# wenyuqing/panacea

Hardware: NVIDIA H100
Metric: UNet denoise-steps/s (6-view x 8-frame latent, CFG-doubled eps-eval + guidance + Euler update) (higher is better)
Workload: dtype bf16

## Files before the change

panacea_b200/csrc/attn_fa.cu:

```cuda
#include "common.cuh"
#include "ptx.cuh"
#include "operand.cuh"
#include "../../include/panacea_b200.h"

namespace pn {

constexpr int FA_THREADS = 288;
constexpr int FA_TILE_BYTES = 128 * 128;
constexpr int FA_XTILE_BYTES = 128 * 32;
constexpr int FA_MAX_KEYS = 128;

template <int D>
struct FaL {
  static constexpr int STAGES = 3;
  static constexpr int XB = D == 64 ? 0 : FA_XTILE_BYTES;
  static constexpr int Q = 0;
  static constexpr int QX = FA_TILE_BYTES;
  static constexpr int KV = FA_TILE_BYTES + XB;
  static constexpr int STAGE_BYTES = 2 * FA_TILE_BYTES + 2 * XB;
  static constexpr int BAR = KV + STAGES * STAGE_BYTES;
  static constexpr int TOTAL = BAR + 128 + 1024;
};

struct FaParams {
  CUtensorMap mapQ;
  CUtensorMap mapK;
  CUtensorMap mapV;
  CUtensorMap mapQx, mapKx, mapVx;
  int heads;
  int F, H, V, W;
  int qw, qh, tiles_x, tiles_y;
  int tiles_per_group;
  int kw, kh, kv_rows, kv_yblocks;
  int kv_views[8][2];
  int kv_view_count[8];
  int kv_frame_div;
  float scale_log2;
  __nv_bfloat16* out;
  long long out_ld;
};

template <int D>
__global__ void __launch_bounds__(FA_THREADS, 1) attn_fa_kernel(const __grid_constant__ FaParams p) {
  using L = FaL<D>;
  constexpr int STAGES = L::STAGES;
  extern __shared__ uint8_t smem_raw[];
  uint8_t* smem = smem_align1024(smem_raw);
  uint64_t* bars = reinterpret_cast<uint64_t*>(smem + L::BAR);
  uint64_t* q_full = bars;
  uint64_t* kv_full = bars + 1;
  uint64_t* kv_empty = bars + 1 + STAGES;

  const int warp = threadIdx.x >> 5;
  const int lane = threadIdx.x & 31;

  {
    uint4* z = reinterpret_cast<uint4*>(smem);
    for (int i = threadIdx.x; i < L::BAR / 16; i += FA_THREADS) z[i] = make_uint4(0, 0, 0, 0);
    fence_proxy_async_smem();
  }
  if (threadIdx.x == 0) {
    mbar_init(q_full, 1);
    for (int i = 0; i < STAGES; ++i) { mbar_init(&kv_full[i], 1); mbar_init(&kv_empty[i], 2); }
    fence_barrier_init();
  }
  __syncthreads();

  int item = blockIdx.x;
  const int ti = item % p.tiles_per_group; item /= p.tiles_per_group;
  const int head = item % p.heads; item /= p.heads;
  const int view = item % p.V;
  const int frame = item / p.V;
  const int nblk = p.kv_view_count[view] * p.kv_yblocks;

  if (warp == 8) {
    const uint32_t q_bytes = (uint32_t)(p.qw * p.qh) * (D == 80 ? 160u : 128u);
    const uint32_t kv_bytes = (uint32_t)p.kv_rows * (D == 80 ? 160u : 128u);
    if (elect_one()) {
      tma_prefetch_desc(&p.mapQ);
      tma_prefetch_desc(&p.mapK);
      tma_prefetch_desc(&p.mapV);
      mbar_arrive_expect_tx(q_full, q_bytes);
      const int x0 = (ti % p.tiles_x) * p.qw, y0 = (ti / p.tiles_x) * p.qh;
      tma_load_5d(smem + L::Q, &p.mapQ, q_full, head * D, x0, view, y0, frame);
      if (D == 80) tma_load_5d(smem + L::QX, &p.mapQx, q_full, head * D + 64, x0, view, y0, frame);
    }
    const int kv_frame = frame / p.kv_frame_div;
    int vi = 0, yb = 0;
    for (int j = 0; j < nblk; ++j) {
      const int st = j % STAGES;
      const int kvv = p.kv_views[view][vi];
      mbar_wait(&kv_empty[st], (uint32_t)(((j / STAGES) & 1) ^ 1));
      if (elect_one()) {
        uint8_t* sK = smem + L::KV + st * L::STAGE_BYTES;
        mbar_arrive_expect_tx(&kv_full[st], 2 * kv_bytes);
        tma_load_5d(sK, &p.mapK, &kv_full[st], head * D, 0, kvv, yb * p.kh, kv_frame);
        tma_load_5d(sK + FA_TILE_BYTES, &p.mapV, &kv_full[st], head * D, 0, kvv, yb * p.kh, kv_frame);
        if (D == 80) {
          tma_load_5d(sK + 2 * FA_TILE_BYTES, &p.mapKx, &kv_full[st], head * D + 64, 0, kvv, yb * p.kh, kv_frame);
          tma_load_5d(sK + 2 * FA_TILE_BYTES + L::XB, &p.mapVx, &kv_full[st], head * D + 64, 0, kvv, yb * p.kh, kv_frame);
        }
      }
      if (++yb == p.kv_yblocks) { yb = 0; ++vi; }
    }
    return;
  }

  const int wg = warp >> 2;
  const int quad = lane & 3;
  const uint32_t base = smem_u32(smem);
  const uint64_t dQ = wgmma_desc(base + L::Q + wg * 64 * 128, 16, 1024, kSw128);
  const uint64_t dQx = wgmma_desc(base + L::QX + wg * 64 * 32, 16, 256, kSw32);
  const uint64_t dK0 = wgmma_desc(base + L::KV, 16, 1024, kSw128);
  const uint64_t dV0 = wgmma_desc(base + L::KV + FA_TILE_BYTES, 1024, 1024, kSw128);
  const uint64_t dKx0 = wgmma_desc(base + L::KV + 2 * FA_TILE_BYTES, 16, 256, kSw32);
  const uint64_t dVx0 = wgmma_desc(base + L::KV + 2 * FA_TILE_BYTES + L::XB, 256, 256, kSw32);
  constexpr uint64_t STAGE_STEP = L::STAGE_BYTES >> 4;
  const float c = p.scale_log2;
  const bool mask = p.kv_rows < FA_MAX_KEYS;

  float o[32], ox[8];
#pragma unroll
  for (int i = 0; i < 32; ++i) o[i] = 0.f;
#pragma unroll
  for (int i = 0; i < 8; ++i) ox[i] = 0.f;
  float m_run[2] = {-INFINITY, -INFINITY}, l_run[2] = {0.f, 0.f};

  mbar_wait(q_full, 0);
  for (int j = 0; j < nblk; ++j) {
    const int st = j % STAGES;
    mbar_wait(&kv_full[st], (uint32_t)((j / STAGES) & 1));
    float s[64];
    wgmma_fence();
#pragma unroll
    for (int k = 0; k < 4; ++k) wgmma_ss<128>(s, dQ + 2 * k, dK0 + STAGE_STEP * st + 2 * k, k > 0 ? 1u : 0u);
    if (D == 80) wgmma_ss<128>(s, dQx, dKx0 + STAGE_STEP * st, 1u);
    wgmma_commit();
    wgmma_wait<0>();
    wgmma_fence_regs(s);

    float mx[2] = {-INFINITY, -INFINITY};
#pragma unroll
    for (int jj = 0; jj < 16; ++jj) {
#pragma unroll
      for (int e = 0; e < 4; ++e) {
        float v = s[4 * jj + e] * c;
        if (mask && 8 * jj + 2 * quad + (e & 1) >= p.kv_rows) v = -INFINITY;
        s[4 * jj + e] = v;
        mx[e >> 1] = fmaxf(mx[e >> 1], v);
      }
    }
    float alpha[2];
#pragma unroll
    for (int h = 0; h < 2; ++h) {
      mx[h] = fmaxf(mx[h], __shfl_xor_sync(0xffffffffu, mx[h], 1));
      mx[h] = fmaxf(mx[h], __shfl_xor_sync(0xffffffffu, mx[h], 2));
      const float m_new = fmaxf(m_run[h], mx[h]);
      alpha[h] = ex2_approx(m_run[h] - m_new);
      m_run[h] = m_new;
    }
    float rs[2] = {0.f, 0.f};
    uint32_t pa[8][4];
#pragma unroll
    for (int jj = 0; jj < 16; ++jj) {
#pragma unroll
      for (int h = 0; h < 2; ++h) {
        const float e0 = ex2_approx(s[4 * jj + 2 * h] - m_run[h]);
        const float e1 = ex2_approx(s[4 * jj + 2 * h + 1] - m_run[h]);
        rs[h] += e0 + e1;
        pa[jj >> 1][(jj & 1) * 2 + h] = pack_bf16x2(e0, e1);
      }
    }
#pragma unroll
    for (int h = 0; h < 2; ++h) l_run[h] = l_run[h] * alpha[h] + rs[h];
#pragma unroll
    for (int jj = 0; jj < 8; ++jj) {
#pragma unroll
      for (int e = 0; e < 4; ++e) o[4 * jj + e] *= alpha[e >> 1];
    }
    if (D == 80) {
#pragma unroll
      for (int e = 0; e < 8; ++e) ox[e] *= alpha[(e >> 1) & 1];
    }

    wgmma_fence();
#pragma unroll
    for (int kk = 0; kk < 8; ++kk) {
      wgmma_rs_tb<64>(o, pa[kk], dV0 + STAGE_STEP * st + kk * (2048 >> 4), 1u);
      if (D == 80) wgmma_rs_tb<16>(ox, pa[kk], dVx0 + STAGE_STEP * st + kk * (512 >> 4), 1u);
    }
    wgmma_commit();
    wgmma_wait<0>();
    wgmma_fence_regs(o);
    if (D == 80) wgmma_fence_regs(ox);
    if ((threadIdx.x & 127) == 0) mbar_arrive(&kv_empty[st]);
  }

#pragma unroll
  for (int h = 0; h < 2; ++h) {
    float l = l_run[h];
    l += __shfl_xor_sync(0xffffffffu, l, 1);
    l += __shfl_xor_sync(0xffffffffu, l, 2);
    const float inv = 1.f / l;
    const int row = wg * 64 + (warp & 3) * 16 + (lane >> 2) + 8 * h;
    const int yy = row / p.qw, xx = row - yy * p.qw;
    const int x = (ti % p.tiles_x) * p.qw + xx, y = (ti / p.tiles_x) * p.qh + yy;
    if (row >= p.qw * p.qh || x >= p.W || y >= p.H) continue;
    const long long token = (((long long)frame * p.H + y) * p.V + view) * p.W + x;
    __nv_bfloat16* dst = p.out + token * p.out_ld + head * D + 2 * quad;
#pragma unroll
    for (int jj = 0; jj < 8; ++jj)
      *reinterpret_cast<uint32_t*>(dst + 8 * jj) = pack_bf16x2(o[4 * jj + 2 * h] * inv, o[4 * jj + 2 * h + 1] * inv);
    if (D == 80) {
#pragma unroll
      for (int jj = 0; jj < 2; ++jj)
        *reinterpret_cast<uint32_t*>(dst + 64 + 8 * jj) = pack_bf16x2(ox[4 * jj + 2 * h] * inv, ox[4 * jj + 2 * h + 1] * inv);
    }
  }
}

}

using namespace pn;

extern "C" int pn_attention(const pn_attn_args* a, int operand_mode, void* stream_v) {
  PN_OPERAND_MODES(Modes, operand_mode, "pn_attention", PN_OPERAND_BF16, PN_OPERAND_SPLIT3, PN_OPERAND_F32);
  if (operand_mode != PN_OPERAND_BF16) return attention_f32(a, operand_mode, stream_v);
  if (a == nullptr) return fail(PN_ERR_INVALID, "pn_attention: null args");
  PN_REQUIRE(a->q && a->k && a->v && a->out, "pn_attention: null tensor pointer");
  PN_REQUIRE(a->head_dim == 64 || a->head_dim == 80, "pn_attention: head_dim %d unsupported (64 or 80)", a->head_dim);
  const int FA_D = a->head_dim;
  PN_REQUIRE(a->heads > 0 && a->F > 0 && a->H > 0 && a->V > 0 && a->V <= 8 && a->W > 0, "pn_attention: bad query geometry");
  PN_REQUIRE(a->Hk > 0 && a->Vk > 0 && a->Vk <= 8 && a->Wk > 0 && a->kv_frame_div > 0, "pn_attention: bad key geometry");
  PN_REQUIRE(a->q_ld % 8 == 0 && a->kv_ld % 8 == 0 && a->out_ld % 8 == 0, "pn_attention: token strides must be multiples of 8");
  PN_REQUIRE(a->q_ld >= a->heads * FA_D && a->kv_ld >= a->heads * FA_D && a->out_ld >= a->heads * FA_D,
             "pn_attention: token stride smaller than heads*64");

  FaParams p;
  std::memset(&p, 0, sizeof(p));
  p.heads = a->heads;
  p.F = (int)a->F; p.H = (int)a->H; p.V = (int)a->V; p.W = (int)a->W;
  p.qw = (int)(a->W <= 128 ? a->W : 128);
  p.qh = 128 / p.qw;
  if (p.qh > a->H) p.qh = (int)a->H;
  if (p.qh < 1) p.qh = 1;
  p.tiles_x = (int)((a->W + p.qw - 1) / p.qw);
  p.tiles_y = (int)((a->H + p.qh - 1) / p.qh);
  PN_REQUIRE(a->Wk <= FA_MAX_KEYS, "pn_attention: key view width %lld > %d unsupported", (long long)a->Wk, FA_MAX_KEYS);
  p.kw = (int)a->Wk;
  int kh = FA_MAX_KEYS / p.kw;
  if (kh > a->Hk) kh = (int)a->Hk;
  while (kh > 1 && (a->Hk % kh) != 0) --kh;
  p.kh = kh;
  p.kv_rows = p.kw * p.kh;
  p.kv_yblocks = (int)(a->Hk / p.kh);
  for (int v = 0; v < a->V; ++v) {
    const int cnt = a->kv_view_count[v];
    PN_REQUIRE(cnt >= 1 && cnt <= 2, "pn_attention: kv_view_count[%d]=%d must be 1 or 2", v, cnt);
    p.kv_view_count[v] = cnt;
    for (int i = 0; i < cnt; ++i) {
      PN_REQUIRE(a->kv_views[v][i] >= 0 && a->kv_views[v][i] < a->Vk, "pn_attention: kv view out of range");
      p.kv_views[v][i] = a->kv_views[v][i];
    }
  }
  p.kv_frame_div = a->kv_frame_div;
  p.scale_log2 = a->scale * 1.4426950408889634f;
  p.out = reinterpret_cast<__nv_bfloat16*>(a->out);
  p.out_ld = a->out_ld;

  const uint64_t chq = (uint64_t)a->heads * FA_D;
  {
    const uint64_t dims[5] = {chq, (uint64_t)a->W, (uint64_t)a->V, (uint64_t)a->H, (uint64_t)a->F};
    const uint64_t ld = (uint64_t)a->q_ld;
    const uint64_t str[4] = {ld, ld * a->W, ld * a->W * a->V, ld * a->W * a->V * a->H};
    const uint32_t box[5] = {64u, (uint32_t)p.qw, 1u, (uint32_t)p.qh, 1u};
    int rc = cached_tmap_bf16(&p.mapQ, a->q, 5, dims, str, box, 128);
    if (rc != PN_OK) return rc;
    if (FA_D == 80) {
      const uint32_t boxx[5] = {16u, (uint32_t)p.qw, 1u, (uint32_t)p.qh, 1u};
      rc = cached_tmap_bf16(&p.mapQx, a->q, 5, dims, str, boxx, 32);
      if (rc != PN_OK) return rc;
    }
  }
  {
    const uint64_t Fk = (uint64_t)((a->F + a->kv_frame_div - 1) / a->kv_frame_div);
    const uint64_t dims[5] = {chq, (uint64_t)a->Wk, (uint64_t)a->Vk, (uint64_t)a->Hk, Fk};
    const uint64_t ld = (uint64_t)a->kv_ld;
    const uint64_t str[4] = {ld, ld * a->Wk, ld * a->Wk * a->Vk, ld * a->Wk * a->Vk * a->Hk};
    const uint32_t box[5] = {64u, (uint32_t)p.kw, 1u, (uint32_t)p.kh, 1u};
    int rc = cached_tmap_bf16(&p.mapK, a->k, 5, dims, str, box, 128);
    if (rc != PN_OK) return rc;
    rc = cached_tmap_bf16(&p.mapV, a->v, 5, dims, str, box, 128);
    if (rc != PN_OK) return rc;
    if (FA_D == 80) {
      const uint32_t boxx[5] = {16u, (uint32_t)p.kw, 1u, (uint32_t)p.kh, 1u};
      rc = cached_tmap_bf16(&p.mapKx, a->k, 5, dims, str, boxx, 32);
      if (rc != PN_OK) return rc;
      rc = cached_tmap_bf16(&p.mapVx, a->v, 5, dims, str, boxx, 32);
      if (rc != PN_OK) return rc;
    }
  }
  p.tiles_per_group = p.tiles_x * p.tiles_y;
  const long long items = (long long)p.tiles_per_group * a->heads * a->V * a->F;
  PN_REQUIRE(items > 0 && items < (1ll << 31), "pn_attention: too many query tiles");
  void (*kern)(FaParams) = FA_D == 80 ? attn_fa_kernel<80> : attn_fa_kernel<64>;
  const size_t smem_total = FA_D == 80 ? FaL<80>::TOTAL : FaL<64>::TOTAL;
  {
    const int rc = ensure_dyn_smem(reinterpret_cast<const void*>(kern), smem_total);
    if (rc != PN_OK) return rc;
  }
  kern<<<(unsigned)items, FA_THREADS, smem_total, reinterpret_cast<cudaStream_t>(stream_v)>>>(p);
  PN_CHECK_CUDA(cudaGetLastError());
  return PN_OK;
}
```

panacea_b200/csrc/ptx.cuh:

```cuda
#pragma once
#include <cstdint>
#include <cuda.h>
#include <cuda_runtime.h>
#include <cuda_bf16.h>

namespace pn {

__device__ __forceinline__ uint32_t smem_u32(const void* p) {
  return static_cast<uint32_t>(__cvta_generic_to_shared(p));
}
__device__ __forceinline__ uint32_t lane_id() { return threadIdx.x & 31; }

__device__ __forceinline__ bool elect_one() {
  uint32_t pred = 0;
  asm volatile(
      "{\n"
      ".reg .pred P;\n"
      "elect.sync _|P, 0xffffffff;\n"
      "selp.u32 %0, 1, 0, P;\n"
      "}\n"
      : "=r"(pred));
  return pred != 0;
}

__device__ __forceinline__ void mbar_init(uint64_t* bar, uint32_t count) {
  asm volatile("mbarrier.init.shared::cta.b64 [%0], %1;" ::"r"(smem_u32(bar)), "r"(count) : "memory");
}
__device__ __forceinline__ void fence_barrier_init() {
  asm volatile("fence.mbarrier_init.release.cluster;" ::: "memory");
}
__device__ __forceinline__ void fence_proxy_async_smem() {
  asm volatile("fence.proxy.async.shared::cta;" ::: "memory");
}
__device__ __forceinline__ void mbar_arrive_expect_tx(uint64_t* bar, uint32_t bytes) {
  asm volatile("mbarrier.arrive.expect_tx.shared::cta.b64 _, [%0], %1;" ::"r"(smem_u32(bar)), "r"(bytes)
               : "memory");
}
__device__ __forceinline__ void mbar_arrive(uint64_t* bar) {
  asm volatile("mbarrier.arrive.shared::cta.b64 _, [%0];" ::"r"(smem_u32(bar)) : "memory");
}
__device__ __forceinline__ bool mbar_try_wait(uint64_t* bar, uint32_t parity) {
  uint32_t ok;
  asm volatile(
      "{\n"
      ".reg .pred p;\n"
      "mbarrier.try_wait.parity.shared::cta.b64 p, [%1], %2;\n"
      "selp.u32 %0, 1, 0, p;\n"
      "}\n"
      : "=r"(ok)
      : "r"(smem_u32(bar)), "r"(parity)
      : "memory");
  return ok != 0;
}
__device__ __forceinline__ void mbar_wait(uint64_t* bar, uint32_t parity) {
  if (mbar_try_wait(bar, parity)) return;
  uint32_t spins = 0;
  while (!mbar_try_wait(bar, parity)) {
    if (++spins > 200000000u) __trap();
  }
}

__device__ __forceinline__ void tma_prefetch_desc(const CUtensorMap* m) {
  asm volatile("prefetch.tensormap [%0];" ::"l"(reinterpret_cast<uint64_t>(m)) : "memory");
}
__device__ __forceinline__ void tma_load_2d(void* dst, const CUtensorMap* m, uint64_t* bar, int c0, int c1) {
  asm volatile(
      "cp.async.bulk.tensor.2d.shared::cluster.global.mbarrier::complete_tx::bytes [%0], [%1, {%3, %4}], [%2];"
      ::"r"(smem_u32(dst)), "l"(reinterpret_cast<uint64_t>(m)), "r"(smem_u32(bar)), "r"(c0), "r"(c1)
      : "memory");
}
__device__ __forceinline__ void tma_load_3d(void* dst, const CUtensorMap* m, uint64_t* bar, int c0, int c1,
                                            int c2) {
  asm volatile(
      "cp.async.bulk.tensor.3d.shared::cluster.global.mbarrier::complete_tx::bytes [%0], [%1, {%3, %4, %5}], "
      "[%2];" ::"r"(smem_u32(dst)),
      "l"(reinterpret_cast<uint64_t>(m)), "r"(smem_u32(bar)), "r"(c0), "r"(c1), "r"(c2)
      : "memory");
}
__device__ __forceinline__ void tma_load_4d(void* dst, const CUtensorMap* m, uint64_t* bar, int c0, int c1,
                                            int c2, int c3) {
  asm volatile(
      "cp.async.bulk.tensor.4d.shared::cluster.global.mbarrier::complete_tx::bytes [%0], [%1, {%3, %4, %5, "
      "%6}], [%2];" ::"r"(smem_u32(dst)),
      "l"(reinterpret_cast<uint64_t>(m)), "r"(smem_u32(bar)), "r"(c0), "r"(c1), "r"(c2), "r"(c3)
      : "memory");
}
__device__ __forceinline__ void tma_load_stage_if(bool pred, uint64_t* bar, uint32_t bytes, void* dst_a, const CUtensorMap* map_a,
                                                  int a0, int a1, int a2, int a3, void* dst_b, const CUtensorMap* map_b, int b0,
                                                  int b1) {
  asm volatile(
      "{\n"
      ".reg .pred p;\n"
      "setp.ne.b32 p, %0, 0;\n"
      "@p mbarrier.arrive.expect_tx.shared::cta.b64 _, [%1], %2;\n"
      "@p cp.async.bulk.tensor.4d.shared::cluster.global.mbarrier::complete_tx::bytes [%3], [%4, {%5, %6, %7, %8}], [%1];\n"
      "@p cp.async.bulk.tensor.2d.shared::cluster.global.mbarrier::complete_tx::bytes [%9], [%10, {%11, %12}], [%1];\n"
      "}\n"
      ::"r"((uint32_t)pred), "r"(smem_u32(bar)), "r"(bytes), "r"(smem_u32(dst_a)), "l"(reinterpret_cast<uint64_t>(map_a)),
      "r"(a0), "r"(a1), "r"(a2), "r"(a3), "r"(smem_u32(dst_b)), "l"(reinterpret_cast<uint64_t>(map_b)), "r"(b0), "r"(b1)
      : "memory");
}
__device__ __forceinline__ void tma_store_2d(const CUtensorMap* m, const void* src, int c0, int c1) {
  asm volatile("cp.async.bulk.tensor.2d.global.shared::cta.bulk_group [%0, {%2, %3}], [%1];"
               ::"l"(reinterpret_cast<uint64_t>(m)), "r"(smem_u32(src)), "r"(c0), "r"(c1) : "memory");
}
__device__ __forceinline__ void bulk_commit() { asm volatile("cp.async.bulk.commit_group;" ::: "memory"); }
__device__ __forceinline__ void bulk_wait_read_all() { asm volatile("cp.async.bulk.wait_group.read 0;" ::: "memory"); }
__device__ __forceinline__ void bulk_wait_all() { asm volatile("cp.async.bulk.wait_group 0;" ::: "memory"); }
__device__ __forceinline__ void named_barrier_sync(uint32_t id, uint32_t threads) {
  asm volatile("bar.sync %0, %1;" ::"r"(id), "r"(threads) : "memory");
}
__device__ __forceinline__ void tma_load_5d(void* dst, const CUtensorMap* m, uint64_t* bar, int c0, int c1,
                                            int c2, int c3, int c4) {
  asm volatile(
      "cp.async.bulk.tensor.5d.shared::cluster.global.mbarrier::complete_tx::bytes [%0], [%1, {%3, %4, %5, "
      "%6, %7}], [%2];" ::"r"(smem_u32(dst)),
      "l"(reinterpret_cast<uint64_t>(m)), "r"(smem_u32(bar)), "r"(c0), "r"(c1), "r"(c2), "r"(c3), "r"(c4)
      : "memory");
}


__device__ __forceinline__ void wgmma_fence() { asm volatile("wgmma.fence.sync.aligned;" ::: "memory"); }
__device__ __forceinline__ void wgmma_commit() { asm volatile("wgmma.commit_group.sync.aligned;" ::: "memory"); }
template <int N>
__device__ __forceinline__ void wgmma_wait() { asm volatile("wgmma.wait_group.sync.aligned %0;" ::"n"(N) : "memory"); }
template <int R>
__device__ __forceinline__ void wgmma_fence_regs(float (&d)[R]) {
#pragma unroll
  for (int i = 0; i < R; ++i) asm volatile("" : "+f"(d[i])::"memory");
}

__device__ __forceinline__ uint64_t wgmma_desc(uint32_t saddr, uint32_t lbo_bytes, uint32_t sbo_bytes, uint32_t layout) {
  uint64_t d = 0;
  d |= static_cast<uint64_t>((saddr & 0x3FFFF) >> 4);
  d |= static_cast<uint64_t>((lbo_bytes >> 4) & 0x3FFF) << 16;
  d |= static_cast<uint64_t>((sbo_bytes >> 4) & 0x3FFF) << 32;
  d |= static_cast<uint64_t>(layout) << 62;
  return d;
}
constexpr uint32_t kSw128 = 1, kSw32 = 3;

template <int N>
__device__ __forceinline__ void wgmma_ss(float (&d)[N / 2], uint64_t a_desc, uint64_t b_desc, uint32_t scale_d);
template <int N>
__device__ __forceinline__ void wgmma_rs_tb(float (&d)[N / 2], const uint32_t (&a)[4], uint64_t b_desc, uint32_t scale_d);

template <>
__device__ __forceinline__ void wgmma_ss<32>(float (&d)[16], uint64_t a_desc, uint64_t b_desc, uint32_t scale_d) {
  asm volatile(
      "{\n.reg .pred p;\nsetp.ne.b32 p, %18, 0;\n"
      "wgmma.mma_async.sync.aligned.m64n32k16.f32.bf16.bf16 {%0, %1, %2, %3, %4, %5, %6, %7, %8, %9, %10, %11, %12, %13, %14, %15}, %16, %17, p, 1, 1, 0, 0;\n}\n"
      : "+f"(d[0]), "+f"(d[1]), "+f"(d[2]), "+f"(d[3]), "+f"(d[4]), "+f"(d[5]), "+f"(d[6]), "+f"(d[7]), "+f"(d[8]), "+f"(d[9]), "+f"(d[10]), "+f"(d[11]), "+f"(d[12]), "+f"(d[13]), "+f"(d[14]), "+f"(d[15])
      : "l"(a_desc), "l"(b_desc), "r"(scale_d));
}

template <>
__device__ __forceinline__ void wgmma_ss<64>(float (&d)[32], uint64_t a_desc, uint64_t b_desc, uint32_t scale_d) {
  asm volatile(
      "{\n.reg .pred p;\nsetp.ne.b32 p, %34, 0;\n"
      "wgmma.mma_async.sync.aligned.m64n64k16.f32.bf16.bf16 {%0, %1, %2, %3, %4, %5, %6, %7, %8, %9, %10, %11, %12, %13, %14, %15, %16, %17, %18, %19, %20, %21, %22, %23, %24, %25, %26, %27, %28, %29, %30, %31}, %32, %33, p, 1, 1, 0, 0;\n}\n"
      : "+f"(d[0]), "+f"(d[1]), "+f"(d[2]), "+f"(d[3]), "+f"(d[4]), "+f"(d[5]), "+f"(d[6]), "+f"(d[7]), "+f"(d[8]), "+f"(d[9]), "+f"(d[10]), "+f"(d[11]), "+f"(d[12]), "+f"(d[13]), "+f"(d[14]), "+f"(d[15]), "+f"(d[16]), "+f"(d[17]), "+f"(d[18]), "+f"(d[19]), "+f"(d[20]), "+f"(d[21]), "+f"(d[22]), "+f"(d[23]), "+f"(d[24]), "+f"(d[25]), "+f"(d[26]), "+f"(d[27]), "+f"(d[28]), "+f"(d[29]), "+f"(d[30]), "+f"(d[31])
      : "l"(a_desc), "l"(b_desc), "r"(scale_d));
}

template <>
__device__ __forceinline__ void wgmma_ss<128>(float (&d)[64], uint64_t a_desc, uint64_t b_desc, uint32_t scale_d) {
  asm volatile(
      "{\n.reg .pred p;\nsetp.ne.b32 p, %66, 0;\n"
      "wgmma.mma_async.sync.aligned.m64n128k16.f32.bf16.bf16 {%0, %1, %2, %3, %4, %5, %6, %7, %8, %9, %10, %11, %12, %13, %14, %15, %16, %17, %18, %19, %20, %21, %22, %23, %24, %25, %26, %27, %28, %29, %30, %31, %32, %33, %34, %35, %36, %37, %38, %39, %40, %41, %42, %43, %44, %45, %46, %47, %48, %49, %50, %51, %52, %53, %54, %55, %56, %57, %58, %59, %60, %61, %62, %63}, %64, %65, p, 1, 1, 0, 0;\n}\n"
      : "+f"(d[0]), "+f"(d[1]), "+f"(d[2]), "+f"(d[3]), "+f"(d[4]), "+f"(d[5]), "+f"(d[6]), "+f"(d[7]), "+f"(d[8]), "+f"(d[9]), "+f"(d[10]), "+f"(d[11]), "+f"(d[12]), "+f"(d[13]), "+f"(d[14]), "+f"(d[15]), "+f"(d[16]), "+f"(d[17]), "+f"(d[18]), "+f"(d[19]), "+f"(d[20]), "+f"(d[21]), "+f"(d[22]), "+f"(d[23]), "+f"(d[24]), "+f"(d[25]), "+f"(d[26]), "+f"(d[27]), "+f"(d[28]), "+f"(d[29]), "+f"(d[30]), "+f"(d[31]), "+f"(d[32]), "+f"(d[33]), "+f"(d[34]), "+f"(d[35]), "+f"(d[36]), "+f"(d[37]), "+f"(d[38]), "+f"(d[39]), "+f"(d[40]), "+f"(d[41]), "+f"(d[42]), "+f"(d[43]), "+f"(d[44]), "+f"(d[45]), "+f"(d[46]), "+f"(d[47]), "+f"(d[48]), "+f"(d[49]), "+f"(d[50]), "+f"(d[51]), "+f"(d[52]), "+f"(d[53]), "+f"(d[54]), "+f"(d[55]), "+f"(d[56]), "+f"(d[57]), "+f"(d[58]), "+f"(d[59]), "+f"(d[60]), "+f"(d[61]), "+f"(d[62]), "+f"(d[63])
      : "l"(a_desc), "l"(b_desc), "r"(scale_d));
}

template <>
__device__ __forceinline__ void wgmma_ss<160>(float (&d)[80], uint64_t a_desc, uint64_t b_desc, uint32_t scale_d) {
  asm volatile(
      "{\n.reg .pred p;\nsetp.ne.b32 p, %82, 0;\n"
      "wgmma.mma_async.sync.aligned.m64n160k16.f32.bf16.bf16 {%0, %1, %2, %3, %4, %5, %6, %7, %8, %9, %10, %11, %12, %13, %14, %15, %16, %17, %18, %19, %20, %21, %22, %23, %24, %25, %26, %27, %28, %29, %30, %31, %32, %33, %34, %35, %36, %37, %38, %39, %40, %41, %42, %43, %44, %45, %46, %47, %48, %49, %50, %51, %52, %53, %54, %55, %56, %57, %58, %59, %60, %61, %62, %63, %64, %65, %66, %67, %68, %69, %70, %71, %72, %73, %74, %75, %76, %77, %78, %79}, %80, %81, p, 1, 1, 0, 0;\n}\n"
      : "+f"(d[0]), "+f"(d[1]), "+f"(d[2]), "+f"(d[3]), "+f"(d[4]), "+f"(d[5]), "+f"(d[6]), "+f"(d[7]), "+f"(d[8]), "+f"(d[9]), "+f"(d[10]), "+f"(d[11]), "+f"(d[12]), "+f"(d[13]), "+f"(d[14]), "+f"(d[15]), "+f"(d[16]), "+f"(d[17]), "+f"(d[18]), "+f"(d[19]), "+f"(d[20]), "+f"(d[21]), "+f"(d[22]), "+f"(d[23]), "+f"(d[24]), "+f"(d[25]), "+f"(d[26]), "+f"(d[27]), "+f"(d[28]), "+f"(d[29]), "+f"(d[30]), "+f"(d[31]), "+f"(d[32]), "+f"(d[33]), "+f"(d[34]), "+f"(d[35]), "+f"(d[36]), "+f"(d[37]), "+f"(d[38]), "+f"(d[39]), "+f"(d[40]), "+f"(d[41]), "+f"(d[42]), "+f"(d[43]), "+f"(d[44]), "+f"(d[45]), "+f"(d[46]), "+f"(d[47]), "+f"(d[48]), "+f"(d[49]), "+f"(d[50]), "+f"(d[51]), "+f"(d[52]), "+f"(d[53]), "+f"(d[54]), "+f"(d[55]), "+f"(d[56]), "+f"(d[57]), "+f"(d[58]), "+f"(d[59]), "+f"(d[60]), "+f"(d[61]), "+f"(d[62]), "+f"(d[63]), "+f"(d[64]), "+f"(d[65]), "+f"(d[66]), "+f"(d[67]), "+f"(d[68]), "+f"(d[69]), "+f"(d[70]), "+f"(d[71]), "+f"(d[72]), "+f"(d[73]), "+f"(d[74]), "+f"(d[75]), "+f"(d[76]), "+f"(d[77]), "+f"(d[78]), "+f"(d[79])
      : "l"(a_desc), "l"(b_desc), "r"(scale_d));
}

template <>
__device__ __forceinline__ void wgmma_rs_tb<16>(float (&d)[8], const uint32_t (&a)[4], uint64_t b_desc, uint32_t scale_d) {
  asm volatile(
      "{\n.reg .pred p;\nsetp.ne.b32 p, %13, 0;\n"
      "wgmma.mma_async.sync.aligned.m64n16k16.f32.bf16.bf16 {%0, %1, %2, %3, %4, %5, %6, %7}, {%8, %9, %10, %11}, %12, p, 1, 1, 1;\n}\n"
      : "+f"(d[0]), "+f"(d[1]), "+f"(d[2]), "+f"(d[3]), "+f"(d[4]), "+f"(d[5]), "+f"(d[6]), "+f"(d[7])
      : "r"(a[0]), "r"(a[1]), "r"(a[2]), "r"(a[3]), "l"(b_desc), "r"(scale_d));
}

template <>
__device__ __forceinline__ void wgmma_rs_tb<64>(float (&d)[32], const uint32_t (&a)[4], uint64_t b_desc, uint32_t scale_d) {
  asm volatile(
      "{\n.reg .pred p;\nsetp.ne.b32 p, %37, 0;\n"
      "wgmma.mma_async.sync.aligned.m64n64k16.f32.bf16.bf16 {%0, %1, %2, %3, %4, %5, %6, %7, %8, %9, %10, %11, %12, %13, %14, %15, %16, %17, %18, %19, %20, %21, %22, %23, %24, %25, %26, %27, %28, %29, %30, %31}, {%32, %33, %34, %35}, %36, p, 1, 1, 1;\n}\n"
      : "+f"(d[0]), "+f"(d[1]), "+f"(d[2]), "+f"(d[3]), "+f"(d[4]), "+f"(d[5]), "+f"(d[6]), "+f"(d[7]), "+f"(d[8]), "+f"(d[9]), "+f"(d[10]), "+f"(d[11]), "+f"(d[12]), "+f"(d[13]), "+f"(d[14]), "+f"(d[15]), "+f"(d[16]), "+f"(d[17]), "+f"(d[18]), "+f"(d[19]), "+f"(d[20]), "+f"(d[21]), "+f"(d[22]), "+f"(d[23]), "+f"(d[24]), "+f"(d[25]), "+f"(d[26]), "+f"(d[27]), "+f"(d[28]), "+f"(d[29]), "+f"(d[30]), "+f"(d[31])
      : "r"(a[0]), "r"(a[1]), "r"(a[2]), "r"(a[3]), "l"(b_desc), "r"(scale_d));
}

__device__ __forceinline__ float ex2_approx(float x) {
  float y;
  asm("ex2.approx.ftz.f32 %0, %1;" : "=f"(y) : "f"(x));
  return y;
}
__device__ __forceinline__ float rcp_approx(float x) {
  float y;
  asm("rcp.approx.ftz.f32 %0, %1;" : "=f"(y) : "f"(x));
  return y;
}
__device__ __forceinline__ uint8_t* smem_align1024(uint8_t* base) {
  return base + ((1024u - (smem_u32(base) & 1023u)) & 1023u);
}
__device__ __forceinline__ uint32_t pack_bf16x2(float lo, float hi) {
  __nv_bfloat162 v = __floats2bfloat162_rn(lo, hi);
  return *reinterpret_cast<uint32_t*>(&v);
}


__device__ __forceinline__ float geglu_f32(float value, float gate) {
  const float t = fabsf(gate);
  float qp = fmaf(5.204588524e-04f, t, -7.397512440e-03f);
  qp = fmaf(qp, t, 5.2561238408e-02f);
  qp = fmaf(qp, t, 4.592546821e-01f);
  qp = fmaf(qp, t, 1.1510913372f);
  const float e = ex2_approx(-(qp * t));
  const float r = fmaf(e, -0.5f, 0.5f);
  return value * fmaf(gate, 0.5f, t * r);
}

__device__ __forceinline__ float silu(float x) { return x * rcp_approx(1.0f + ex2_approx(-1.4426950408889634f * x)); }

}
```

Measured before the change: 4.064.

## Pipeline S and PV wgmma, size key block to kv_rows, add row-major Q tiling

Restructures the flash-attention consumer loop so the QK^T wgmma for block j is issued together with the PV wgmma for block j-1, overlapping tensor-core work with softmax. Templates the kernel on key-block width N, chosen from kv_rows, so narrow key views no longer compute padded 128-wide tiles. Adds a row-major Q tiling mode, loaded with several small TMA boxes, that fills 128-row query tiles when the spatial tiling would leave them partly empty. Also folds the softmax scale into an FMA and applies masking only to the tail groups. In exchange it holds more live registers and compiles eight kernel variants per head dim.

```diff
diff --git a/panacea_b200/csrc/attn_fa.cu b/panacea_b200/csrc/attn_fa.cu
--- a/panacea_b200/csrc/attn_fa.cu
+++ b/panacea_b200/csrc/attn_fa.cu
@@ -9,6 +9,7 @@
 constexpr int FA_TILE_BYTES = 128 * 128;
 constexpr int FA_XTILE_BYTES = 128 * 32;
 constexpr int FA_MAX_KEYS = 128;
+constexpr int FA_QBOX = 8;
 
 template <int D>
 struct FaL {
@@ -29,6 +30,7 @@
   CUtensorMap mapQx, mapKx, mapVx;
   int heads;
   int F, H, V, W;
+  int q_rowmajor;
   int qw, qh, tiles_x, tiles_y;
   int tiles_per_group;
   int kw, kh, kv_rows, kv_yblocks;
@@ -40,10 +42,13 @@
   long long out_ld;
 };
 
-template <int D>
+template <int D, int N>
 __global__ void __launch_bounds__(FA_THREADS, 1) attn_fa_kernel(const __grid_constant__ FaParams p) {
+  static_assert(N % 16 == 0 && N >= 16 && N <= FA_MAX_KEYS, "a key block is a whole number of K = 16 steps of P V");
   using L = FaL<D>;
   constexpr int STAGES = L::STAGES;
+  constexpr int GROUPS = N / 8;
+  constexpr int KSTEPS = N / 16;
   extern __shared__ uint8_t smem_raw[];
   uint8_t* smem = smem_align1024(smem_raw);
   uint64_t* bars = reinterpret_cast<uint64_t*>(smem + L::BAR);
@@ -74,16 +79,27 @@
   const int nblk = p.kv_view_count[view] * p.kv_yblocks;
 
   if (warp == 8) {
-    const uint32_t q_bytes = (uint32_t)(p.qw * p.qh) * (D == 80 ? 160u : 128u);
-    const uint32_t kv_bytes = (uint32_t)p.kv_rows * (D == 80 ? 160u : 128u);
+    const uint32_t row_bytes = D == 80 ? 160u : 128u;
+    const uint32_t kv_bytes = (uint32_t)p.kv_rows * row_bytes;
     if (elect_one()) {
       tma_prefetch_desc(&p.mapQ);
       tma_prefetch_desc(&p.mapK);
       tma_prefetch_desc(&p.mapV);
-      mbar_arrive_expect_tx(q_full, q_bytes);
-      const int x0 = (ti % p.tiles_x) * p.qw, y0 = (ti / p.tiles_x) * p.qh;
-      tma_load_5d(smem + L::Q, &p.mapQ, q_full, head * D, x0, view, y0, frame);
-      if (D == 80) tma_load_5d(smem + L::QX, &p.mapQx, q_full, head * D + 64, x0, view, y0, frame);
+      if (p.q_rowmajor) {
+        const int t0 = ti * 128;
+        const int rows = min(128, p.H * p.W - t0);
+        mbar_arrive_expect_tx(q_full, (uint32_t)rows * row_bytes);
+        for (int r = 0; r < rows; r += FA_QBOX) {
+          const int y = (t0 + r) / p.W, x = t0 + r - y * p.W;
+          tma_load_5d(smem + L::Q + r * 128, &p.mapQ, q_full, head * D, x, view, y, frame);
+          if (D == 80) tma_load_5d(smem + L::QX + r * 32, &p.mapQx, q_full, head * D + 64, x, view, y, frame);
+        }
+      } else {
+        mbar_arrive_expect_tx(q_full, (uint32_t)(p.qw * p.qh) * row_bytes);
+        const int x0 = (ti % p.tiles_x) * p.qw, y0 = (ti / p.tiles_x) * p.qh;
+        tma_load_5d(smem + L::Q, &p.mapQ, q_full, head * D, x0, view, y0, frame);
+        if (D == 80) tma_load_5d(smem + L::QX, &p.mapQx, q_full, head * D + 64, x0, view, y0, frame);
+      }
     }
     const int kv_frame = frame / p.kv_frame_div;
     int vi = 0, yb = 0;
@@ -117,7 +133,7 @@
   const uint64_t dVx0 = wgmma_desc(base + L::KV + 2 * FA_TILE_BYTES + L::XB, 256, 256, kSw32);
   constexpr uint64_t STAGE_STEP = L::STAGE_BYTES >> 4;
   const float c = p.scale_log2;
-  const bool mask = p.kv_rows < FA_MAX_KEYS;
+  const bool mask = p.kv_rows < N;
 
   float o[32], ox[8];
 #pragma unroll
@@ -125,76 +141,103 @@
 #pragma unroll
   for (int i = 0; i < 8; ++i) ox[i] = 0.f;
   float m_run[2] = {-INFINITY, -INFINITY}, l_run[2] = {0.f, 0.f};
-
-  mbar_wait(q_full, 0);
-  for (int j = 0; j < nblk; ++j) {
-    const int st = j % STAGES;
-    mbar_wait(&kv_full[st], (uint32_t)((j / STAGES) & 1));
-    float s[64];
-    wgmma_fence();
-#pragma unroll
-    for (int k = 0; k < 4; ++k) wgmma_ss<128>(s, dQ + 2 * k, dK0 + STAGE_STEP * st + 2 * k, k > 0 ? 1u : 0u);
-    if (D == 80) wgmma_ss<128>(s, dQx, dKx0 + STAGE_STEP * st, 1u);
+  float s[N / 2];
+  uint32_t pa[KSTEPS][4];
+  float alpha[2];
+
+  auto issue_s = [&](int st) {
+#pragma unroll
+    for (int k = 0; k < 4; ++k) wgmma_ss<N>(s, dQ + 2 * k, dK0 + STAGE_STEP * st + 2 * k, k > 0 ? 1u : 0u);
+    if (D == 80) wgmma_ss<N>(s, dQx, dKx0 + STAGE_STEP * st, 1u);
     wgmma_commit();
-    wgmma_wait<0>();
-    wgmma_fence_regs(s);
-
+  };
+  auto issue_pv = [&](int st) {
+#pragma unroll
+    for (int kk = 0; kk < KSTEPS; ++kk) {
+      wgmma_rs_tb<64>(o, pa[kk], dV0 + STAGE_STEP * st + kk * (2048 >> 4), 1u);
+      if (D == 80) wgmma_rs_tb<16>(ox, pa[kk], dVx0 + STAGE_STEP * st + kk * (512 >> 4), 1u);
+    }
+    wgmma_commit();
+  };
+  auto softmax = [&]() {
     float mx[2] = {-INFINITY, -INFINITY};
 #pragma unroll
-    for (int jj = 0; jj < 16; ++jj) {
+    for (int jj = 0; jj < GROUPS; ++jj) {
 #pragma unroll
       for (int e = 0; e < 4; ++e) {
-        float v = s[4 * jj + e] * c;
-        if (mask && 8 * jj + 2 * quad + (e & 1) >= p.kv_rows) v = -INFINITY;
-        s[4 * jj + e] = v;
-        mx[e >> 1] = fmaxf(mx[e >> 1], v);
+        if (jj >= GROUPS - 2 && mask && 8 * jj + 2 * quad + (e & 1) >= p.kv_rows) s[4 * jj + e] = -INFINITY;
+        mx[e >> 1] = fmaxf(mx[e >> 1], s[4 * jj + e]);
       }
     }
-    float alpha[2];
+    float mc[2];
 #pragma unroll
     for (int h = 0; h < 2; ++h) {
       mx[h] = fmaxf(mx[h], __shfl_xor_sync(0xffffffffu, mx[h], 1));
       mx[h] = fmaxf(mx[h], __shfl_xor_sync(0xffffffffu, mx[h], 2));
       const float m_new = fmaxf(m_run[h], mx[h]);
-      alpha[h] = ex2_approx(m_run[h] - m_new);
+      alpha[h] = ex2_approx((m_run[h] - m_new) * c);
       m_run[h] = m_new;
+      mc[h] = m_new * c;
     }
     float rs[2] = {0.f, 0.f};
-    uint32_t pa[8][4];
-#pragma unroll
-    for (int jj = 0; jj < 16; ++jj) {
-#pragma unroll
-      for (int h = 0; h < 2; ++h) {
-        const float e0 = ex2_approx(s[4 * jj + 2 * h] - m_run[h]);
-        const float e1 = ex2_approx(s[4 * jj + 2 * h + 1] - m_run[h]);
-        rs[h] += e0 + e1;
-        pa[jj >> 1][(jj & 1) * 2 + h] = pack_bf16x2(e0, e1);
+#pragma unroll
+    for (int jj = 0; jj < GROUPS; ++jj) {
+#pragma unroll
+      for (int e = 0; e < 4; ++e) {
+        const float x = fmaf(s[4 * jj + e], c, -mc[e >> 1]);
+        const float v = ex2_approx(x);
+        s[4 * jj + e] = v;
+        rs[e >> 1] += v;
       }
     }
 #pragma unroll
     for (int h = 0; h < 2; ++h) l_run[h] = l_run[h] * alpha[h] + rs[h];
-#pragma unroll
-    for (int jj = 0; jj < 8; ++jj) {
-#pragma unroll
-      for (int e = 0; e < 4; ++e) o[4 * jj + e] *= alpha[e >> 1];
-    }
+  };
+  auto rescale_and_pack = [&]() {
+#pragma unroll
+    for (int i = 0; i < 32; ++i) o[i] *= alpha[(i >> 1) & 1];
     if (D == 80) {
 #pragma unroll
-      for (int e = 0; e < 8; ++e) ox[e] *= alpha[(e >> 1) & 1];
-    }
-
-    wgmma_fence();
-#pragma unroll
-    for (int kk = 0; kk < 8; ++kk) {
-      wgmma_rs_tb<64>(o, pa[kk], dV0 + STAGE_STEP * st + kk * (2048 >> 4), 1u);
-      if (D == 80) wgmma_rs_tb<16>(ox, pa[kk], dVx0 + STAGE_STEP * st + kk * (512 >> 4), 1u);
-    }
-    wgmma_commit();
-    wgmma_wait<0>();
+      for (int i = 0; i < 8; ++i) ox[i] *= alpha[(i >> 1) & 1];
+    }
+#pragma unroll
+    for (int jj = 0; jj < GROUPS; ++jj) {
+#pragma unroll
+      for (int h = 0; h < 2; ++h) pa[jj >> 1][(jj & 1) * 2 + h] = pack_bf16x2(s[4 * jj + 2 * h], s[4 * jj + 2 * h + 1]);
+    }
+  };
+  auto pv_retired = [&](int st) {
     wgmma_fence_regs(o);
     if (D == 80) wgmma_fence_regs(ox);
+#pragma unroll
+    for (int kk = 0; kk < KSTEPS; ++kk) wgmma_fence_regs(pa[kk]);
     if ((threadIdx.x & 127) == 0) mbar_arrive(&kv_empty[st]);
-  }
+  };
+
+  mbar_wait(q_full, 0);
+  mbar_wait(&kv_full[0], 0);
+  wgmma_fence();
+  issue_s(0);
+  wgmma_wait<0>();
+  wgmma_fence_regs(s);
+  softmax();
+  rescale_and_pack();
+  for (int j = 1; j < nblk; ++j) {
+    const int st = j % STAGES, prev = (j - 1) % STAGES;
+    mbar_wait(&kv_full[st], (uint32_t)((j / STAGES) & 1));
+    wgmma_fence();
+    issue_s(st);
+    issue_pv(prev);
+    wgmma_wait<0>();
+    wgmma_fence_regs(s);
+    pv_retired(prev);
+    softmax();
+    rescale_and_pack();
+  }
+  wgmma_fence();
+  issue_pv((nblk - 1) % STAGES);
+  wgmma_wait<0>();
+  pv_retired((nblk - 1) % STAGES);
 
 #pragma unroll
   for (int h = 0; h < 2; ++h) {
@@ -203,9 +246,18 @@
     l += __shfl_xor_sync(0xffffffffu, l, 2);
     const float inv = 1.f / l;
     const int row = wg * 64 + (warp & 3) * 16 + (lane >> 2) + 8 * h;
-    const int yy = row / p.qw, xx = row - yy * p.qw;
-    const int x = (ti % p.tiles_x) * p.qw + xx, y = (ti / p.tiles_x) * p.qh + yy;
-    if (row >= p.qw * p.qh || x >= p.W || y >= p.H) continue;
+    int x, y;
+    if (p.q_rowmajor) {
+      const int t = ti * 128 + row;
+      y = t / p.W;
+      x = t - y * p.W;
+    } else {
+      if (row >= p.qw * p.qh) continue;
+      const int yy = row / p.qw, xx = row - yy * p.qw;
+      x = (ti % p.tiles_x) * p.qw + xx;
+      y = (ti / p.tiles_x) * p.qh + yy;
+    }
+    if (x >= p.W || y >= p.H) continue;
     const long long token = (((long long)frame * p.H + y) * p.V + view) * p.W + x;
     __nv_bfloat16* dst = p.out + token * p.out_ld + head * D + 2 * quad;
 #pragma unroll
@@ -218,6 +270,11 @@
     }
   }
 }
+
+template <int D>
+void (*const fa_kernels[FA_MAX_KEYS / 16])(FaParams) = {attn_fa_kernel<D, 16>, attn_fa_kernel<D, 32>, attn_fa_kernel<D, 48>,
+                                                        attn_fa_kernel<D, 64>, attn_fa_kernel<D, 80>, attn_fa_kernel<D, 96>,
+                                                        attn_fa_kernel<D, 112>, attn_fa_kernel<D, 128>};
 
 }
 
@@ -246,6 +303,7 @@
   if (p.qh < 1) p.qh = 1;
   p.tiles_x = (int)((a->W + p.qw - 1) / p.qw);
   p.tiles_y = (int)((a->H + p.qh - 1) / p.qh);
+  p.q_rowmajor = a->W % FA_QBOX == 0 && a->W < 128 && p.qw * p.qh < 128 && a->H > p.qh;
   PN_REQUIRE(a->Wk <= FA_MAX_KEYS, "pn_attention: key view width %lld > %d unsupported", (long long)a->Wk, FA_MAX_KEYS);
   p.kw = (int)a->Wk;
   int kh = FA_MAX_KEYS / p.kw;
@@ -273,11 +331,12 @@
     const uint64_t dims[5] = {chq, (uint64_t)a->W, (uint64_t)a->V, (uint64_t)a->H, (uint64_t)a->F};
     const uint64_t ld = (uint64_t)a->q_ld;
     const uint64_t str[4] = {ld, ld * a->W, ld * a->W * a->V, ld * a->W * a->V * a->H};
-    const uint32_t box[5] = {64u, (uint32_t)p.qw, 1u, (uint32_t)p.qh, 1u};
+    const uint32_t bw = p.q_rowmajor ? FA_QBOX : p.qw, bh = p.q_rowmajor ? 1 : p.qh;
+    const uint32_t box[5] = {64u, bw, 1u, bh, 1u};
     int rc = cached_tmap_bf16(&p.mapQ, a->q, 5, dims, str, box, 128);
     if (rc != PN_OK) return rc;
     if (FA_D == 80) {
-      const uint32_t boxx[5] = {16u, (uint32_t)p.qw, 1u, (uint32_t)p.qh, 1u};
+      const uint32_t boxx[5] = {16u, bw, 1u, bh, 1u};
       rc = cached_tmap_bf16(&p.mapQx, a->q, 5, dims, str, boxx, 32);
       if (rc != PN_OK) return rc;
     }
@@ -300,10 +359,11 @@
       if (rc != PN_OK) return rc;
     }
   }
-  p.tiles_per_group = p.tiles_x * p.tiles_y;
+  p.tiles_per_group = p.q_rowmajor ? (int)((a->H * a->W + 127) / 128) : p.tiles_x * p.tiles_y;
   const long long items = (long long)p.tiles_per_group * a->heads * a->V * a->F;
   PN_REQUIRE(items > 0 && items < (1ll << 31), "pn_attention: too many query tiles");
-  void (*kern)(FaParams) = FA_D == 80 ? attn_fa_kernel<80> : attn_fa_kernel<64>;
+  const int n_idx = (p.kv_rows + 15) / 16 - 1;
+  void (*kern)(FaParams) = FA_D == 80 ? fa_kernels<80>[n_idx] : fa_kernels<64>[n_idx];
   const size_t smem_total = FA_D == 80 ? FaL<80>::TOTAL : FaL<64>::TOTAL;
   {
     const int rc = ensure_dyn_smem(reinterpret_cast<const void*>(kern), smem_total);
diff --git a/panacea_b200/csrc/ptx.cuh b/panacea_b200/csrc/ptx.cuh
--- a/panacea_b200/csrc/ptx.cuh
+++ b/panacea_b200/csrc/ptx.cuh
@@ -129,6 +129,11 @@
 #pragma unroll
   for (int i = 0; i < R; ++i) asm volatile("" : "+f"(d[i])::"memory");
 }
+template <int R>
+__device__ __forceinline__ void wgmma_fence_regs(uint32_t (&a)[R]) {
+#pragma unroll
+  for (int i = 0; i < R; ++i) asm volatile("" : "+r"(a[i])::"memory");
+}
 
 __device__ __forceinline__ uint64_t wgmma_desc(uint32_t saddr, uint32_t lbo_bytes, uint32_t sbo_bytes, uint32_t layout) {
   uint64_t d = 0;
@@ -146,6 +151,15 @@
 __device__ __forceinline__ void wgmma_rs_tb(float (&d)[N / 2], const uint32_t (&a)[4], uint64_t b_desc, uint32_t scale_d);
 
 template <>
+__device__ __forceinline__ void wgmma_ss<16>(float (&d)[8], uint64_t a_desc, uint64_t b_desc, uint32_t scale_d) {
+  asm volatile(
+      "{\n.reg .pred p;\nsetp.ne.b32 p, %10, 0;\n"
+      "wgmma.mma_async.sync.aligned.m64n16k16.f32.bf16.bf16 {%0, %1, %2, %3, %4, %5, %6, %7}, %8, %9, p, 1, 1, 0, 0;\n}\n"
+      : "+f"(d[0]), "+f"(d[1]), "+f"(d[2]), "+f"(d[3]), "+f"(d[4]), "+f"(d[5]), "+f"(d[6]), "+f"(d[7])
+      : "l"(a_desc), "l"(b_desc), "r"(scale_d));
+}
+
+template <>
 __device__ __forceinline__ void wgmma_ss<32>(float (&d)[16], uint64_t a_desc, uint64_t b_desc, uint32_t scale_d) {
   asm volatile(
       "{\n.reg .pred p;\nsetp.ne.b32 p, %18, 0;\n"
@@ -155,11 +169,47 @@
 }
 
 template <>
+__device__ __forceinline__ void wgmma_ss<48>(float (&d)[24], uint64_t a_desc, uint64_t b_desc, uint32_t scale_d) {
+  asm volatile(
+      "{\n.reg .pred p;\nsetp.ne.b32 p, %26, 0;\n"
+      "wgmma.mma_async.sync.aligned.m64n48k16.f32.bf16.bf16 {%0, %1, %2, %3, %4, %5, %6, %7, %8, %9, %10, %11, %12, %13, %14, %15, %16, %17, %18, %19, %20, %21, %22, %23}, %24, %25, p, 1, 1, 0, 0;\n}\n"
+      : "+f"(d[0]), "+f"(d[1]), "+f"(d[2]), "+f"(d[3]), "+f"(d[4]), "+f"(d[5]), "+f"(d[6]), "+f"(d[7]), "+f"(d[8]), "+f"(d[9]), "+f"(d[10]), "+f"(d[11]), "+f"(d[12]), "+f"(d[13]), "+f"(d[14]), "+f"(d[15]), "+f"(d[16]), "+f"(d[17]), "+f"(d[18]), "+f"(d[19]), "+f"(d[20]), "+f"(d[21]), "+f"(d[22]), "+f"(d[23])
+      : "l"(a_desc), "l"(b_desc), "r"(scale_d));
+}
+
+template <>
 __device__ __forceinline__ void wgmma_ss<64>(float (&d)[32], uint64_t a_desc, uint64_t b_desc, uint32_t scale_d) {
   asm volatile(
       "{\n.reg .pred p;\nsetp.ne.b32 p, %34, 0;\n"
       "wgmma.mma_async.sync.aligned.m64n64k16.f32.bf16.bf16 {%0, %1, %2, %3, %4, %5, %6, %7, %8, %9, %10, %11, %12, %13, %14, %15, %16, %17, %18, %19, %20, %21, %22, %23, %24, %25, %26, %27, %28, %29, %30, %31}, %32, %33, p, 1, 1, 0, 0;\n}\n"
       : "+f"(d[0]), "+f"(d[1]), "+f"(d[2]), "+f"(d[3]), "+f"(d[4]), "+f"(d[5]), "+f"(d[6]), "+f"(d[7]), "+f"(d[8]), "+f"(d[9]), "+f"(d[10]), "+f"(d[11]), "+f"(d[12]), "+f"(d[13]), "+f"(d[14]), "+f"(d[15]), "+f"(d[16]), "+f"(d[17]), "+f"(d[18]), "+f"(d[19]), "+f"(d[20]), "+f"(d[21]), "+f"(d[22]), "+f"(d[23]), "+f"(d[24]), "+f"(d[25]), "+f"(d[26]), "+f"(d[27]), "+f"(d[28]), "+f"(d[29]), "+f"(d[30]), "+f"(d[31])
+      : "l"(a_desc), "l"(b_desc), "r"(scale_d));
+}
+
+template <>
+__device__ __forceinline__ void wgmma_ss<80>(float (&d)[40], uint64_t a_desc, uint64_t b_desc, uint32_t scale_d) {
+  asm volatile(
+      "{\n.reg .pred p;\nsetp.ne.b32 p, %42, 0;\n"
+      "wgmma.mma_async.sync.aligned.m64n80k16.f32.bf16.bf16 {%0, %1, %2, %3, %4, %5, %6, %7, %8, %9, %10, %11, %12, %13, %14, %15, %16, %17, %18, %19, %20, %21, %22, %23, %24, %25, %26, %27, %28, %29, %30, %31, %32, %33, %34, %35, %36, %37, %38, %39}, %40, %41, p, 1, 1, 0, 0;\n}\n"
+      : "+f"(d[0]), "+f"(d[1]), "+f"(d[2]), "+f"(d[3]), "+f"(d[4]), "+f"(d[5]), "+f"(d[6]), "+f"(d[7]), "+f"(d[8]), "+f"(d[9]), "+f"(d[10]), "+f"(d[11]), "+f"(d[12]), "+f"(d[13]), "+f"(d[14]), "+f"(d[15]), "+f"(d[16]), "+f"(d[17]), "+f"(d[18]), "+f"(d[19]), "+f"(d[20]), "+f"(d[21]), "+f"(d[22]), "+f"(d[23]), "+f"(d[24]), "+f"(d[25]), "+f"(d[26]), "+f"(d[27]), "+f"(d[28]), "+f"(d[29]), "+f"(d[30]), "+f"(d[31]), "+f"(d[32]), "+f"(d[33]), "+f"(d[34]), "+f"(d[35]), "+f"(d[36]), "+f"(d[37]), "+f"(d[38]), "+f"(d[39])
+      : "l"(a_desc), "l"(b_desc), "r"(scale_d));
+}
+
+template <>
+__device__ __forceinline__ void wgmma_ss<96>(float (&d)[48], uint64_t a_desc, uint64_t b_desc, uint32_t scale_d) {
+  asm volatile(
+      "{\n.reg .pred p;\nsetp.ne.b32 p, %50, 0;\n"
+      "wgmma.mma_async.sync.aligned.m64n96k16.f32.bf16.bf16 {%0, %1, %2, %3, %4, %5, %6, %7, %8, %9, %10, %11, %12, %13, %14, %15, %16, %17, %18, %19, %20, %21, %22, %23, %24, %25, %26, %27, %28, %29, %30, %31, %32, %33, %34, %35, %36, %37, %38, %39, %40, %41, %42, %43, %44, %45, %46, %47}, %48, %49, p, 1, 1, 0, 0;\n}\n"
+      : "+f"(d[0]), "+f"(d[1]), "+f"(d[2]), "+f"(d[3]), "+f"(d[4]), "+f"(d[5]), "+f"(d[6]), "+f"(d[7]), "+f"(d[8]), "+f"(d[9]), "+f"(d[10]), "+f"(d[11]), "+f"(d[12]), "+f"(d[13]), "+f"(d[14]), "+f"(d[15]), "+f"(d[16]), "+f"(d[17]), "+f"(d[18]), "+f"(d[19]), "+f"(d[20]), "+f"(d[21]), "+f"(d[22]), "+f"(d[23]), "+f"(d[24]), "+f"(d[25]), "+f"(d[26]), "+f"(d[27]), "+f"(d[28]), "+f"(d[29]), "+f"(d[30]), "+f"(d[31]), "+f"(d[32]), "+f"(d[33]), "+f"(d[34]), "+f"(d[35]), "+f"(d[36]), "+f"(d[37]), "+f"(d[38]), "+f"(d[39]), "+f"(d[40]), "+f"(d[41]), "+f"(d[42]), "+f"(d[43]), "+f"(d[44]), "+f"(d[45]), "+f"(d[46]), "+f"(d[47])
+      : "l"(a_desc), "l"(b_desc), "r"(scale_d));
+}
+
+template <>
+__device__ __forceinline__ void wgmma_ss<112>(float (&d)[56], uint64_t a_desc, uint64_t b_desc, uint32_t scale_d) {
+  asm volatile(
+      "{\n.reg .pred p;\nsetp.ne.b32 p, %58, 0;\n"
+      "wgmma.mma_async.sync.aligned.m64n112k16.f32.bf16.bf16 {%0, %1, %2, %3, %4, %5, %6, %7, %8, %9, %10, %11, %12, %13, %14, %15, %16, %17, %18, %19, %20, %21, %22, %23, %24, %25, %26, %27, %28, %29, %30, %31, %32, %33, %34, %35, %36, %37, %38, %39, %40, %41, %42, %43, %44, %45, %46, %47, %48, %49, %50, %51, %52, %53, %54, %55}, %56, %57, p, 1, 1, 0, 0;\n}\n"
+      : "+f"(d[0]), "+f"(d[1]), "+f"(d[2]), "+f"(d[3]), "+f"(d[4]), "+f"(d[5]), "+f"(d[6]), "+f"(d[7]), "+f"(d[8]), "+f"(d[9]), "+f"(d[10]), "+f"(d[11]), "+f"(d[12]), "+f"(d[13]), "+f"(d[14]), "+f"(d[15]), "+f"(d[16]), "+f"(d[17]), "+f"(d[18]), "+f"(d[19]), "+f"(d[20]), "+f"(d[21]), "+f"(d[22]), "+f"(d[23]), "+f"(d[24]), "+f"(d[25]), "+f"(d[26]), "+f"(d[27]), "+f"(d[28]), "+f"(d[29]), "+f"(d[30]), "+f"(d[31]), "+f"(d[32]), "+f"(d[33]), "+f"(d[34]), "+f"(d[35]), "+f"(d[36]), "+f"(d[37]), "+f"(d[38]), "+f"(d[39]), "+f"(d[40]), "+f"(d[41]), "+f"(d[42]), "+f"(d[43]), "+f"(d[44]), "+f"(d[45]), "+f"(d[46]), "+f"(d[47]), "+f"(d[48]), "+f"(d[49]), "+f"(d[50]), "+f"(d[51]), "+f"(d[52]), "+f"(d[53]), "+f"(d[54]), "+f"(d[55])
       : "l"(a_desc), "l"(b_desc), "r"(scale_d));
 }
 
```

New measurement: 4.245, median of 6. 1.04x the previous value.
